# Denopia/canonical-k-mer-hash-table

Measured on AMD Instinct MI355X. Metric: k-mers/s inserted (canonical) + achieved HBM GB/s, 1/2/4/8 MI355X, higher is better.
Workload: dtype u64; 1 GPU; C2: synthetic 10000000 x 150 bp reads/GPU, k=31, -m 2 -s 200000000; reads_per_gpu=10000000, read_len=150, k=31, genome=50000000, table=-m 2 -s 200000000, parallelism=single

## Files before the change

canonical-k-mer-hash-table_amd/csrc/kc_count_impl.h:

```cpp
#pragma once
#include <algorithm>
#include <cstdlib>
#include <cstring>

#include "kc_common.h"

namespace kc {

static __constant__ uint64_t c_bf_seeds[MAX_NH] = {2411, 3253, 1061, 1129, 2269, 7309, 3491, 8237, 6359, 8779};

template <int W>
DEV bool table_insert(const TableView& tv, const uint64_t (&tk)[W], uint64_t add = 1) {
    constexpr int S = BUCKET_WORDS / (W + 1);
    const uint64_t region = region_of(tk[0], tv.R);
    uint32_t b = bucket_in_region(tk[0], tv.R);
    for (int probe = 0; probe < BPR; probe++) {
        uint64_t* bk = tv.buckets + (region * BPR + b) * BUCKET_WORDS;
        uint64_t w0[S];
        if constexpr (W == 1) {
            const uint4* b4 = reinterpret_cast<const uint4*>(bk);
#pragma unroll
            for (int q = 0; q < S / 2; q++) {
                uint4 v = b4[q];
                w0[2 * q] = ((uint64_t)v.y << 32) | v.x;
// ... 208 lines not shown
    return all;
}

DEV void block_add4(unsigned long long v0, unsigned long long v1, unsigned long long v2, unsigned long long v3,
                    unsigned long long* d0, unsigned long long* d1, unsigned long long* d2,
                    unsigned long long* d3) {
    __shared__ unsigned long long s_red[4][16];
    unsigned long long v[4] = {v0, v1, v2, v3};
    const int lane = threadIdx.x & 63, wid = threadIdx.x >> 6;
#pragma unroll
    for (int q = 0; q < 4; q++) {
        unsigned long long x = v[q];
        for (int d = 32; d >= 1; d >>= 1) x += __shfl_xor(x, d, 64);
        if (lane == 0) s_red[q][wid] = x;
    }
    __syncthreads();
    if (threadIdx.x < 4) {
        unsigned long long x = 0;
        for (int w = 0; w < (int)(blockDim.x / 64); w++) x += s_red[threadIdx.x][w];
        unsigned long long* dst = threadIdx.x == 0 ? d0 : threadIdx.x == 1 ? d1 : threadIdx.x == 2 ? d2 : d3;
        if (x && dst) atomicAdd(dst, x);
    }
}

template <int W>
constexpr int run_w() { return run_width(W); }
template <int W>
constexpr int tile_win() { return COUNT_THREADS * run_w<W>(); }
template <int W>
constexpr int scatter_threads() { return scatter_threads_w(W); }
template <int W, int NT>
constexpr int k1_runw() { return NT == scatter_threads_w(W) ? p1_runw(W) : run_w<W>(); }
template <int W, int OW, int NT>
constexpr size_t p1_smem(uint32_t F) { return bin_lds_bytes(F) + (size_t)NT * k1_runw<W, NT>() * 8 * OW; }
template <int W, int NT>
constexpr int k1_stage_words() { return NT * k1_runw<W, NT>() / 32 + W + 3; }
template <int W, int NT>
constexpr size_t p1_stage_smem() { return (size_t)k1_stage_words<W, NT>() * 24; }
template <int W>
constexpr int p2f_threads() { return p2f_threads_w(W); }

template <int W>
DEV bool window_tkey(const PackedView& sv, uint64_t p, const RollConst& rk, uint64_t (&tk)[W]) {
    uint64_t fwd[W], rc[W], key[W];
    if (!extract_window<W>(sv, p, rk, fwd)) return false;
    revcomp<W>(fwd, rk, rc);
    canonical<W>(fwd, rc, key);
    to_tkey<W>(key, tk);
    return true;
}

template <int W, int RUNW = run_w<W>(), class F>
DEV void tile_rolled(const PackedView& sv, uint64_t t0, uint64_t t1, const RollConst& rk, F&& f) {
    const uint64_t r0 = t0 + (uint64_t)threadIdx.x * RUNW, r1 = min(r0 + RUNW, t1);
    if (r0 < r1) {
        const uint64_t ps = r0 >= (uint64_t)(rk.k - 1) ? r0 - (rk.k - 1) : 0;
        roll_run<W, true>(sv, ps, r0, r1, rk, f);
    }
}

template <int W, int MODE>
__global__ __launch_bounds__(COUNT_THREADS) void k_count(PackedView sv, int k, TableView tv, BloomView bf,
                                                         DevCounters* __restrict__ ctr, uint64_t pow5_k,
                                                         uint64_t pow5_km1) {
    constexpr int TW = tile_win<W>();
    const uint64_t M = ctr->stream_len;
    const uint64_t t0 = (uint64_t)blockIdx.x * TW;
// ... 198 lines not shown
            const uint64_t pos = s_spbase + l.sp[b] + (i - lim);
            if (pos < o.spill_cap) {
                uint64_t* r = o.spill + pos * (W + o.rec);
#pragma unroll
                for (int w = 0; w < W; w++) r[w] = key[w];
                if (o.rec) r[W] = 1;
            } else {
                atomicOr(o.overflow, 1ULL);
            }
        }
    }
    __syncthreads();
    for (uint32_t b = tid; b < F; b += NT) {
        l.gbase[b] += l.lim[b];
        l.hist[b] = 0;
    }
    __syncthreads();
    return false;
}

DEV void scatter_seg_init(const PartLds& l, uint32_t b, uint64_t first) {
    l.hist[b] = 0;
    l.lim[b] = 0;
    l.gbase[b] = first;
}
DEV uint64_t scatter_seg_next(const PartLds& l, uint32_t b) { return l.gbase[b] + l.lim[b]; }

struct StoreWords {
    template <int W>
    DEV void operator()(uint64_t* __restrict__ out, uint64_t dst, const uint64_t (&key)[W], uint32_t) const {
#pragma unroll
        for (int w = 0; w < W; w++) ks_store(out + dst * W + w, key[w]);
    }
};
DEV uint64_t region_xlo(uint64_t r, uint64_t R) { return ((r << 32) + R - 1) / R; }
struct StoreRec6 {
    const uint32_t* xlo;
    DEV void operator()(uint64_t* __restrict__ out, uint64_t dst, const uint64_t (&key)[1], uint32_t b) const {
        uint32_t* q = reinterpret_cast<uint32_t*>(out) + (dst >> 1) * 3;
        q[dst & 1] = (uint32_t)key[0];
        reinterpret_cast<uint16_t*>(q + 2)[dst & 1] = (uint16_t)((uint32_t)(key[0] >> 32) - xlo[b]);
    }
};
struct Rec12 {
    int hb, xb;
    DEV uint3 enc(uint64_t t0, uint64_t t1) const {
        const uint32_t x = (uint32_t)(t0 >> 32), d = x & ((1u << xb) - 1);
        const uint32_t hi = ((uint32_t)(t1 >> 32) & ((1u << hb) - 1)) | (uint32_t)((t1 >> 62) & 1) << hb;
        return make_uint3((uint32_t)t0, (uint32_t)t1, hi | d << (hb + 1));
    }
    DEV void dec(uint3 r, uint32_t x0, uint64_t& t0, uint64_t& t1) const {
        const uint32_t x = x0 + (((r.z >> (hb + 1)) - x0) & ((1u << xb) - 1));
        t0 = ((uint64_t)x << 32) | r.x;
        t1 = ((uint64_t)(r.z & ((1u << hb) - 1)) << 32) | r.y | ((uint64_t)((r.z >> hb) & 1) << 62);
    }
};
struct StoreW2 {
    bool rec12;
    Rec12 rc;
    DEV void operator()(uint64_t* __restrict__ out, uint64_t dst, const uint64_t (&key)[2], uint32_t) const {
        if (rec12) {
            reinterpret_cast<uint3*>(out)[dst] = rc.enc(key[0], key[1]);
        } else {
            ks_store(out + dst * 2, key[0]);
            ks_store(out + dst * 2 + 1, key[1]);
        }
    }
};

template <int W, int RUNW, class Bin, class Out, int NT, class Mid = NoMid, class St = StoreWords, class Pre = NoMid>
DEV void scatter_seg(const PartLds& l, uint32_t F, const Bin& bin, const Out& o, uint64_t (&tk)[RUNW][W],
                     bool (&ok)[RUNW], uint64_t* __restrict__ out, Mid&& mid = Mid(),
                     const St& store = St(), Pre&& pre = Pre()) {
    static_assert(NT * RUNW <= 65536, "ranks ride in 16 bits");
    __shared__ unsigned long long s_spbase;
    __shared__ uint32_t s_spills, s_n;
    const int tid = threadIdx.x, lane = tid & 63;
    uint32_t pk[RUNW];
#pragma unroll
    for (int j = 0; j < RUNW; j++) {
        const uint32_t b = bin(tk[j][0]);
        if constexpr (W >= 2) {
            const uint32_t rk = atomicAdd(&l.hist[b], ok[j] ? 1u : 0u);
            pk[j] = ok[j] ? (b << 16) | rk : ~0u;
        } else {
            pk[j] = ok[j] ? (b << 16) | atomicAdd(&l.hist[b], 1u) : ~0u;
        }
    }
    pre();
    __syncthreads();
    if (tid < 64) {
        if (F % 4 == 0) {
            const uint32_t per = (F / 4 + 63) / 64, lo = min(F / 4, lane * per), hi = min(F / 4, lo + per);
            const uint4* h4 = reinterpret_cast<const uint4*>(l.hist);
            uint4* s4 = reinterpret_cast<uint4*>(l.start);
            uint32_t sum = 0;
#pragma unroll 1
            for (uint32_t i = lo; i < hi; i++) {
                const uint4 v = h4[i];
                sum += v.x + v.y + v.z + v.w;
            }
            const uint32_t incl = wave_incl_sum(sum);
            uint32_t run = incl - sum;
#pragma unroll 1
            for (uint32_t i = lo; i < hi; i++) {
                const uint4 v = h4[i];
                s4[i] = make_uint4(run, run + v.x, run + v.x + v.y, run + v.x + v.y + v.z);
                run += v.x + v.y + v.z + v.w;
            }
            if (lane == 63) s_n = incl;
        } else {
            const uint32_t per = (F + 63) / 64, lo = min(F, lane * per), hi = min(F, lo + per);
            uint32_t sum = 0;
#pragma unroll 1
            for (uint32_t i = lo; i < hi; i++) sum += l.hist[i];
            const uint32_t incl = wave_incl_sum(sum);
            uint32_t run = incl - sum;
#pragma unroll 1
            for (uint32_t i = lo; i < hi; i++) {
                l.start[i] = run;
                run += l.hist[i];
            }
            if (lane == 63) s_n = incl;
        }
        if (Out::kSeg && lane == 0) s_spills = 0;
    }
    __syncthreads();
#pragma unroll
    for (int j = 0; j < RUNW; j++)
        if (pk[j] != ~0u) {
            const uint32_t slot = l.start[pk[j] >> 16] + (pk[j] & 0xFFFFu);
#pragma unroll
            for (int w = 0; w < W; w++) l.keys[slot * W + w] = tk[j][w];
        }
    bool spills = false;
#pragma unroll 1
    for (uint32_t b = tid; b < F; b += NT) {
        const uint32_t st = l.start[b], h = l.hist[b];
        const uint64_t g = l.gbase[b] + l.lim[b];
        const uint32_t fit = (uint32_t)min((uint64_t)h, o.room(b, g));
        l.gbase[b] = g - st;
        l.lim[b] = st + fit;
        l.sp[b] = h - fit;
        l.hist[b] = 0;
        spills |= fit < h;
    }
    if (Out::kSeg && spills) s_spills = 1;
    mid();
    __syncthreads();
    if constexpr (Out::kSeg) {
        if (s_spills) {
            const uint32_t last = l.sp[F - 1];
            block_excl_scan_lds<NT>(l.sp, l.sp, F);
            if (tid == 0) s_spbase = atomicAdd(o.spill_n, (unsigned long long)(l.sp[F - 1] + last));
            __syncthreads();
        }
    }
    const uint32_t n = s_n;
    auto emit = [&](uint32_t i, const uint64_t (&key)[W], uint32_t b, uint32_t lim, uint64_t g) {
        if (i < lim) {
            store(out, g + i, key, b);
        } else if constexpr (Out::kSeg) {
            const uint64_t pos = s_spbase + l.sp[b] + (i - lim);
            if (pos < o.spill_cap) {
                uint64_t* r = o.spill + pos * (W + o.rec);
#pragma unroll
                for (int w = 0; w < W; w++) r[w] = key[w];
                if (o.rec) r[W] = 1;
            } else {
                atomicOr(o.overflow, 1ULL);
            }
        }
    };
#pragma unroll 1
    for (uint32_t i0 = tid; i0 < n; i0 += 2 * NT) {
        const uint32_t i1 = i0 + NT;
        const bool has1 = i1 < n;
        uint64_t k0[W], k1[W];
#pragma unroll
        for (int w = 0; w < W; w++) {
            k0[w] = l.keys[i0 * W + w];
            k1[w] = l.keys[(has1 ? i1 : i0) * W + w];
        }
        const uint32_t b0 = bin(k0[0]), b1 = bin(k1[0]);
        const uint32_t lim0 = l.lim[b0], lim1 = l.lim[b1];
        const uint64_t g0 = l.gbase[b0], g1 = l.gbase[b1];
        emit(i0, k0, b0, lim0, g0);
        if (has1) emit(i1, k1, b1, lim1, g1);
    }
}

constexpr bool bloom_mode(int MODE) { return MODE == 3 || MODE == 5; }

constexpr int HT = 64;
template <int OW>
constexpr size_t heavy_smem() { return (size_t)HT * (OW + 1) * 8; }
struct HeavyTab {
    uint64_t* keys;
    uint64_t* cnt;
};
template <int OW>
DEV HeavyTab heavy_tab(uint8_t* p) {
    HeavyTab h;
    h.keys = reinterpret_cast<uint64_t*>(p);
    h.cnt = h.keys + HT * OW;
    return h;
// ... 117 lines not shown
        const uint64_t c = h.cnt[e] & CNT_MASK;
        const bool has = key[0] != EMPTY;
        skew_append<OW, MODE>(pb, ctr, has, key, c);
        const uint64_t nrec = __ballot(has);
        if (threadIdx.x == 0 && nrec) atomicAdd(&ctr->heavy_n, (unsigned long long)__popcll(nrec));
    }
}

DEV bool gated_off(const unsigned long long* gate) { return gate && *gate == 0; }

constexpr int p1_out_words(int W, int MODE) { return MODE == 3 ? 1 : W; }
constexpr int scatter_waves(int NT, int RUNW, int OW, int cap) {
    const int wg = (int)(LDS_BYTES / ((size_t)NT * RUNW * 8 * OW));
    const int w = (wg < 1 ? 1 : wg) * NT / 256;
    return w < 1 ? 1 : w > cap ? cap : w;
}


template <int W, int MODE, bool SCATTER, class Bin, class Out, int NT = COUNT_THREADS>
__global__ __launch_bounds__(NT, scatter_waves(NT, k1_runw<W, NT>(), p1_out_words(W, MODE), 4)) void k_p1(PackedView sv, int k, BloomView bf,
                                                      DevCounters* __restrict__ ctr, PartBufs pb, uint32_t F, Bin bin_arg,
                                                      uint64_t* __restrict__ out, uint64_t pow5_k, uint64_t pow5_km1,
                                                      Out o, const unsigned long long* gate, int count) {
    extern __shared__ __attribute__((aligned(16))) uint8_t smem[];
    const Bin bin = level1_bins(bin_arg);
    constexpr int RUNW = k1_runw<W, NT>(), TW = NT * RUNW;
    constexpr bool COUNTS = !SCATTER || Out::kSeg;
    constexpr bool ROLLED = MODE == 2;
    constexpr int OW = p1_out_words(W, MODE);
    if (gated_off(gate)) return;
    if (gate && !SCATTER && blockIdx.x == 0 && threadIdx.x == 0) atomicAdd(&ctr->part_fallbacks, 1ULL);
    const PartLds l = part_lds(smem, F);
    constexpr bool HEAVY = Out::kSeg && !Bin::kOwner && !ROLLED;
    const HeavyTab ht = heavy_tab<OW>(smem + p1_smem<W, OW, NT>(F));
    if constexpr (HEAVY) {
        heavy_clear(ht, OW);
        for (int i = threadIdx.x; i < HT; i += NT) ht.cnt[i] = 0;
    }
    const int tid = threadIdx.x;
    const uint64_t M = ctr->stream_len;
    const uint64_t per = ((M + pb.nblk1 - 1) / pb.nblk1 + TW - 1) / TW * TW;
    const uint64_t lo = min(M, (uint64_t)blockIdx.x * per), hi = min(M, lo + per);
    constexpr bool STAGE = Out::kSeg && !ROLLED;
    constexpr int SW = k1_stage_words<W, NT>();
    static_assert(!STAGE || SW <= NT, "one stage word per thread");
    uint64_t* st_pk = reinterpret_cast<uint64_t*>(smem + p1_smem<W, OW, NT>(F) + heavy_smem<OW>());
    uint32_t* st_bk = reinterpret_cast<uint32_t*>(st_pk + 2 * SW);
    const uint64_t wlim = M ? ((M - 1) >> 5) + 1 : 0;
    auto stage_word = [&](uint64_t ts, int i, uint64_t& pw, uint32_t& bw) {
        const int64_t w = (int64_t)(ts >> 5) - (W + 1) + i;
        const bool in = w >= 0 && (uint64_t)w <= wlim;
        pw = in ? sv.pk[w] : 0;
        bw = in ? sv.bk[w] : 0;
    };
    if constexpr (STAGE)
        if (lo < hi && tid < SW) stage_word(lo, tid, st_pk[tid], st_bk[tid]);
    int par = 0;
    Out ob = o;
    if constexpr (Out::kSeg) ob.base = (uint64_t)blockIdx.x * o.cap;
    for (uint32_t b = tid; b < F; b += NT) {
        if constexpr (Out::kSeg) {
            scatter_seg_init(l, b, ob.start(b));
        } else {
            l.hist[b] = 0;
            if constexpr (SCATTER) l.gbase[b] = pb.off1[(uint64_t)b * pb.nblk1 + blockIdx.x];
        }
    }
    __syncthreads();
    const RollConst rk = make_roll<W>(k, pow5_k, pow5_km1);
    uint32_t n_win = 0, n_ins = 0;
    for (uint64_t t0 = lo; t0 < hi; t0 += TW) {
        const uint64_t t1 = min(t0 + TW, hi);
        uint64_t tk[RUNW][OW];
        bool ok[RUNW];
        if constexpr (!ROLLED) {
            const uint64_t r0 = t0 + (uint64_t)tid * RUNW;
#pragma unroll
            for (int j = 0; j < RUNW; j++) ok[j] = false;
            auto emit = [&](int j, bool valid, const uint64_t (&fwd)[W], const uint64_t (&rc)[W]) {
// ... 28 lines not shown
                canonical<W>(fwd, rc, key);
                to_tkey<W>(key, t);
                if (!bloom_gate(bf, root, t[0])) return;
                if constexpr (COUNTS) n_ins++;
#pragma unroll
                for (int j = 0; j < RUNW; j++)
                    if (!ok[j]) {
                        ok[j] = true;
#pragma unroll
                        for (int w = 0; w < W; w++) tk[j][w] = t[w];
                        break;
                    }
            });
        }
        if constexpr (SCATTER) {
            if constexpr (Out::kSeg) {
                const bool nxt = STAGE && t0 + TW < hi && tid < SW;
                uint64_t npk = 0;
                uint32_t nbk = 0;
                auto mid = [&]() {
                    if (nxt) {
                        st_pk[(par ^ 1) * SW + tid] = npk;
                        st_bk[(par ^ 1) * SW + tid] = nbk;
                    }
                };
                auto pre = [&]() {
                    if (nxt) stage_word(t0 + TW, tid, npk, nbk);
                };
                if constexpr (OW == 2)
                    scatter_seg<OW, RUNW, Bin, Out, NT>(l, F, bin, ob, tk, ok, out, mid,
                                                        StoreW2{(pb.rec12 & R12_P1) != 0, Rec12{pb.r12_hb, pb.r12_xb1}},
                                                        pre);
                else
                    scatter_seg<OW, RUNW, Bin, Out, NT>(l, F, bin, ob, tk, ok, out, mid, StoreWords(), pre);
                par ^= 1;
            } else {
                scatter_tile<OW, RUNW, Bin, Out, NT>(l, F, bin, ob, tk, ok, out, NoMid());
            }
        } else {
#pragma unroll
            for (int j = 0; j < RUNW; j++)
                if (ok[j]) atomicAdd(&l.hist[bin(tk[j][0])], 1u);
        }
    }
    if constexpr (!SCATTER) {
        __syncthreads();
        for (uint32_t b = tid; b < F; b += NT) pb.hist1[(uint64_t)b * pb.nblk1 + blockIdx.x] = l.hist[b];
    }
    if constexpr (Out::kSeg) {
        __syncthreads();
        for (uint32_t b = tid; b < F; b += NT)
            pb.hist1[(uint64_t)b * pb.nblk1 + blockIdx.x] = (uint32_t)(scatter_seg_next(l, b) - ob.start(b));
    }
    if constexpr (HEAVY) heavy_flush<OW, MODE>(ht, pb, ctr);
    if constexpr (COUNTS)
        if (count) {
            if constexpr (bloom_mode(MODE))
                block_add4(n_win, 0, 0, 0, &ctr->bf_windows, nullptr, nullptr, nullptr);
            else
                block_add4(n_win, Bin::kOwner ? 0 : n_ins, 0, 0, &ctr->windows, &ctr->inserted, nullptr, nullptr);
        }
}

struct DevN {
    const unsigned long long* dn;
    uint64_t cap;
    const unsigned long long* ovf;
// ... 170 lines not shown
            const uint64_t i = t0 + tid + (uint64_t)q * COUNT_THREADS;
            ok[q] = i < hi;
            const uint64_t ii = ok[q] ? i : lo;
#pragma unroll
            for (int w = 0; w < W; w++) tk[q][w] = pb.keys1[ii * W + w];
        }
        if constexpr (SCATTER) {
            scatter_tile<W, RUNW>(l, F, bin, OutExact{}, tk, ok, pb.keys2);
        } else {
#pragma unroll
            for (int q = 0; q < RUNW; q++)
                if (ok[q]) atomicAdd(&l.hist[bin(tk[q][0])], 1u);
        }
    }
    if constexpr (!SCATTER) {
        __syncthreads();
        for (uint32_t b = tid; b < F; b += COUNT_THREADS) pb.hist2[(rbase + b) * pb.B2 + j] = l.hist[b];
    }
}

template <int W, int NT>
constexpr size_t p2f_smem(uint32_t F, uint32_t nseg_max) { return part_smem<W, NT>(F) + (size_t)(nseg_max + 1) * 4; }

template <int W, int NT, int IS = W, bool REC6 = false>
__global__ __launch_bounds__(NT, scatter_waves(NT, run_w<W>(), W, 2048 / NT > 8 ? 8 : 2048 / NT)) void k_p2f(TableView tv, PartBufs pb, DevCounters* __restrict__ ctr,
                                                          int REC) {
    static_assert(!REC6 || W == 1, "6-byte records hold one-word keys");
    extern __shared__ __attribute__((aligned(16))) uint8_t smem[];
    constexpr int RUNW = run_w<W>(), TW = NT * RUNW;
    if (ctr->part_overflow) return;
    const uint32_t F = tv.F2;
    const BinRegion bin{tv.R, tv.f2bits, F - 1, 0};
    const PartLds l = part_lds(smem, F);
    uint32_t* pre = reinterpret_cast<uint32_t*>(smem + part_smem<W, NT>(F));
    const int tid = threadIdx.x;
    const uint32_t c = blockIdx.x / pb.B2, j = blockIdx.x % pb.B2;
    const uint32_t s_lo = (uint32_t)((uint64_t)j * pb.nblk1 / pb.B2);
    const uint32_t nseg = (uint32_t)((uint64_t)(j + 1) * pb.nblk1 / pb.B2) - s_lo;
    const uint64_t seg0 = (uint64_t)c * pb.nblk1 + s_lo;
    const uint32_t B2T = pb.b2t ? pb.b2t : pb.B2, jo = pb.b2off + j;
    const OutSeg o{(uint64_t)B2T * pb.cap2, ((uint64_t)c * F * B2T + jo) * pb.cap2, pb.cap2,
                   pb.spill, pb.spill_cap, &ctr->spill_n, &ctr->part_overflow, REC};
    for (uint32_t i = tid; i <= nseg; i += NT) pre[i] = i < nseg ? pb.hist1[seg0 + i] : 0;
    uint32_t* xlo = pre + nseg + 1;
    if constexpr (REC6)
        for (uint32_t b = tid; b < F; b += NT) xlo[b] = (uint32_t)region_xlo((uint64_t)c * F + b, tv.R);
    for (uint32_t b = tid; b < F; b += NT) scatter_seg_init(l, b, o.start(b));
    __syncthreads();
    block_excl_scan_lds<NT>(pre, pre, nseg + 1);
    const uint32_t total = pre[nseg];
    uint32_t cs = 0, cb = 0, nb = nseg ? pre[1] : 0;
    const bool rin = W == 2 && (pb.rec12 & R12_IN), rout = W == 2 && (pb.rec12 & R12_OUT);
    const uint32_t x0c = rin ? (uint32_t)region_xlo((uint64_t)c * F, tv.R) : 0;
    const uint64_t* sp = pb.keys1 + seg0 * pb.cap1 * IS;
    const uint32_t wpos = (uint32_t)(tid >> 6) * (64 * RUNW) + (tid & 63);
    auto load_tile = [&](uint32_t t0, uint64_t (&tk)[RUNW][W], bool (&ok)[RUNW]) {
#pragma unroll
        for (int q = 0; q < RUNW; q++) {
            const uint32_t i = t0 + wpos + q * 64;
            ok[q] = i < total;
            const uint64_t* src = sp;
            uint64_t item = (seg0 + cs) * pb.cap1;
            if (ok[q]) {
                if (nb <= i) {
                    do {
                        cs++;
                        cb = nb;
// ... 6 lines not shown
            }
            if constexpr (W == 2) {
                const uint64_t off = rin ? item * 12 : item * (8 * IS);
                uint32_t v[4];
                __builtin_memcpy(v, reinterpret_cast<const uint8_t*>(pb.keys1) + off, 16);
                tk[q][0] = v[0] | (uint64_t)v[1] << 32;
                tk[q][1] = v[2] | (uint64_t)v[3] << 32;
                (void)src;
                continue;
            }
#pragma unroll
            for (int w = 0; w < W; w++) tk[q][w] = ks_load(src + w);
        }
    };
    uint64_t tk[RUNW][W];
    bool ok[RUNW];
    if (total) load_tile(0, tk, ok);
    for (uint32_t t0 = 0; t0 < total; t0 += TW) {
        const bool more = t0 + TW < total;
        auto mid = [&]() {
            if (more) load_tile(t0 + TW, tk, ok);
        };
        if constexpr (W == 2) {
            if (rin) {
                const Rec12 r1{pb.r12_hb, pb.r12_xb1};
#pragma unroll
                for (int q = 0; q < RUNW; q++) {
                    const uint3 v = make_uint3((uint32_t)tk[q][0], (uint32_t)(tk[q][0] >> 32), (uint32_t)tk[q][1]);
                    r1.dec(v, x0c, tk[q][0], tk[q][1]);
                }
            }
        }
        if constexpr (REC6) {
            scatter_seg<W, RUNW, BinRegion, OutSeg, NT>(l, F, bin, o, tk, ok, pb.keys2, mid,
                                                        StoreRec6{xlo});
        } else if constexpr (W == 2) {
            scatter_seg<W, RUNW, BinRegion, OutSeg, NT>(l, F, bin, o, tk, ok, pb.keys2, mid,
                                                        StoreW2{rout, Rec12{pb.r12_hb, pb.r12_xb2}});
        } else {
            scatter_seg<W, RUNW, BinRegion, OutSeg, NT>(l, F, bin, o, tk, ok, pb.keys2, mid);
        }
    }
    __syncthreads();
    for (uint32_t b = tid; b < F; b += NT)
        pb.hist2[((uint64_t)c * F + b) * B2T + jo] = (uint32_t)(scatter_seg_next(l, b) - o.start(b));
}

DEV uint32_t lds_chunk(uint32_t b, uint32_t q) { return b * 8 + (q ^ ((b >> 1) & 7)); }
DEV uint64_t* lds_word(uint64_t* lt, uint32_t b, uint32_t word) {
    return lt + lds_chunk(b, word >> 1) * 2 + (word & 1);
}

DEV uint32_t slot_tag(uint64_t t0) { return 1u + (((uint32_t)t0 & 0xFFu) * 255u >> 8); }
DEV uint32_t zero_byte_mask4(uint32_t x) {
    const uint32_t z = ~(((x & 0x7F7F7F7Fu) + 0x7F7F7F7Fu) | x | 0x7F7F7F7Fu);
    return ((z >> 7) * 0x01020408u) >> 24;
}
DEV uint32_t zero_byte_mask8(uint64_t x) {
    return zero_byte_mask4((uint32_t)x) | zero_byte_mask4((uint32_t)(x >> 32)) << 4;
}

DEV void seg_prefix(uint32_t* s_pre, const uint32_t* __restrict__ fill, uint32_t n, uint32_t* s_pp = nullptr) {
    if (threadIdx.x < 64) {
        const uint32_t j = 2 * threadIdx.x;
        const uint32_t a = j < n ? fill[j] : 0, b = j + 1 < n ? fill[j + 1] : 0;
        const uint32_t inc = wave_incl_sum(a + b);
        const uint32_t ex = inc - (a + b);
        if (j < n) s_pre[j] = ex;
// ... 921 lines not shown
    hipLaunchKernelGGL(kh, dim3(pb.nblk1), dim3(COUNT_THREADS), sm1h, s, sym, k, bf, ctr, pb, F, bin, out, pk, pkm1,
                       OutExact{}, gate, count);
    launch_scan(pb.hist1, (uint64_t)F * pb.nblk1, pb.off1, pb.bsum, s, gate);
    hipLaunchKernelGGL(ks, dim3(pb.nblk1), dim3(COUNT_THREADS), sm1, s, sym, k, bf, ctr, pb, F, bin, out, pk, pkm1,
                       OutExact{}, gate, 0);
    return hipGetLastError();
}

template <int W, bool GATE>
static hipError_t insert_spill(TableView t, BloomView bf, DevCounters* ctr, PartBufs pb, hipStream_t s) {
    constexpr int IW = W + 1;
    const BinRegion bin = coarse_bins(t);
    const size_t sm1 = part_smem<IW>(t.F1), sm1h = hist_smem(t.F1);
    hipError_t e;
    if ((e = set_smem(k_p1k<IW, false>, sm1h)) != hipSuccess) return e;
    if ((e = set_smem(k_p1k<IW, true>, sm1)) != hipSuccess) return e;
    const DevN dn{&ctr->spill_n, pb.spill_cap, &ctr->part_overflow};
    hipLaunchKernelGGL((k_p1k<IW, false>), dim3(pb.nblk1), dim3(COUNT_THREADS), sm1h, s, pb.spill, (uint64_t)0, pb,
                       t.F1, bin, ctr, W, dn, IW);
    launch_scan(pb.hist1, (uint64_t)t.F1 * pb.nblk1, pb.off1, pb.bsum, s);
    hipLaunchKernelGGL((k_p1k<IW, true>), dim3(pb.nblk1), dim3(COUNT_THREADS), sm1, s, pb.spill, (uint64_t)0, pb,
                       t.F1, bin, ctr, W, dn, IW);
    return part_levels23<W, true, GATE>(t, ctr, pb, s, nullptr, 0, bf);
}

template <int W>
static hipError_t launch_p2f(TableView t, PartBufs pb, DevCounters* ctr, int rec, hipStream_t s, uint32_t pad = 0) {
    constexpr int NT = p2f_threads<W>(), NH = NT / 2;
    const uint32_t nseg = std::max<uint32_t>(pad, (pb.nblk1 + pb.B2 - 1) / pb.B2);
    hipError_t e;
    const size_t sm = p2f_smem<W, NT>(t.F2, nseg);
    if constexpr (W == 1) {
        if (pb.rec6) {
            if ((e = set_smem(k_p2f<1, NT, 1, true>, sm + (size_t)t.F2 * 4)) != hipSuccess) return e;
            hipLaunchKernelGGL((k_p2f<1, NT, 1, true>), dim3(t.F1 * pb.B2), dim3(NT), sm + (size_t)t.F2 * 4, s, t, pb,
                               ctr, rec);
            return hipGetLastError();
        }
    }
    if (sm <= LDS_BYTES || W <= 2) {
        if ((e = set_smem(k_p2f<W, NT>, sm)) != hipSuccess) return e;
        hipLaunchKernelGGL((k_p2f<W, NT>), dim3(t.F1 * pb.B2), dim3(NT), sm, s, t, pb, ctr, rec);
    } else {
        const size_t smh = p2f_smem<W, NH>(t.F2, nseg);
        if ((e = set_smem(k_p2f<W, NH>, smh)) != hipSuccess) return e;
        hipLaunchKernelGGL((k_p2f<W, NH>), dim3(t.F1 * pb.B2), dim3(NH), smh, s, t, pb, ctr, rec);
    }
    return hipGetLastError();
}

static __global__ void k_batch_begin(DevCounters* ctr) {
    ctr->part_overflow = 0;
    ctr->spill_n = 0;
    ctr->heavy_n = 0;
}
static __global__ void k_batch_end(DevCounters* ctr) {
    if (ctr->part_overflow) return;
    ctr->spilled += ctr->spill_n - ctr->heavy_n;
    ctr->heavy += ctr->heavy_n;
}

static inline void set_rec12_table(PartBufs& pb, const TableView& t, int k) {
    pb.rec12 = 0;
    if (t.R == 0) return;
    const int hb = std::max(0, 2 * k - 96);
    const uint64_t f2 = 1ULL << t.f2bits;
    const int xb1 = span_bits32(((f2 << 32) + t.R - 1) / t.R), xb2 = span_bits32(((1ULL << 32) + t.R - 1) / t.R);
    if (hb + 1 + xb1 <= 32) {
        pb.rec12 |= R12_P1 | R12_IN;
// ... 3 lines not shown
        pb.rec12 |= R12_OUT | R12_L2;
        pb.r12_xb2 = xb2;
    }
    if (pb.rec12) pb.rec12 |= R12_REG;
    pb.r12_hb = hb;
    pb.r12_b2s = 0;
}

template <int W, int MODE>
static hipError_t launch_part_w(PackedView sym, int k, TableView t, BloomView bf, DevCounters* ctr, PartBufs pb,
                                int fresh, hipStream_t s, int phase) {
    constexpr bool GATE3 = MODE == 4;
    if (pb.cap1 == 0) {
        if (!(phase & PH_MAIN)) return hipSuccess;
        hipError_t e = part_level1<W, MODE>(sym, k, bf, ctr, pb, t.F1, coarse_bins(t), pb.keys1, s);
        if (e != hipSuccess) return e;
        return part_levels23<W, false, GATE3>(t, ctr, pb, s, nullptr, fresh, bf);
    }
    hipError_t e;
    const unsigned long long* gate = &ctr->part_overflow;
    pb.rec6 = W == 1 && t.R >= (1ULL << 16);
    if constexpr (W == 2) set_rec12_table(pb, t, k);
    if (phase & PH_L3) {
        PartBufs p3 = pb;
        p3.B2 = pb.b2t;
        p3.b2t = p3.b2off = 0;
        if ((e = launch_p3<W, true, false, GATE3>(t, ctr, p3, nullptr, fresh, s, bf)) != hipSuccess) return e;
    }
    if (phase & (PH_MAIN | PH_L12)) {
    if (!pb.keep_skew) hipLaunchKernelGGL(k_batch_begin, dim3(1), dim3(1), 0, s, ctr);
    const uint64_t pk = pow5_mod54(k), pkm1 = pow5_mod54(k - 1);
    auto k1 = k_p1<W, MODE, true, BinRegion, OutSeg, scatter_threads<W>()>;
    const size_t p1_lds_min = (size_t)p1_tile(W) < 8 * (size_t)t.F1 ? LDS_BYTES / 2 + 16 : 0;
    const size_t sm1 = std::max(p1_lds_min, p1_smem<W, W, scatter_threads<W>()>(t.F1) + heavy_smem<W>() +
                                                p1_stage_smem<W, scatter_threads<W>()>());
    const OutSeg o1{(uint64_t)pb.nblk1 * pb.cap1, 0, pb.cap1, pb.spill, pb.spill_cap, &ctr->spill_n,
                    &ctr->part_overflow, 1};
    bool wide = false;
    if constexpr (W == 2) {
        if (p1_wide(W, t.F1)) {
            wide = true;
            auto kw = k_p1<W, MODE, true, BinRegion, OutSeg, P1_WIDE_THREADS>;
            const size_t smw = p1_smem<W, W, P1_WIDE_THREADS>(t.F1) + heavy_smem<W>() + p1_stage_smem<W, P1_WIDE_THREADS>();
            if ((e = set_smem(kw, smw)) != hipSuccess) return e;
            hipLaunchKernelGGL(kw, dim3(pb.nblk1), dim3(P1_WIDE_THREADS), smw, s, sym, k, bf, ctr, pb, t.F1,
                               coarse_bins(t), pb.keys1, pk, pkm1, o1, (const unsigned long long*)nullptr, 1);
        }
    }
    if (!wide) {
        if ((e = set_smem(k1, sm1)) != hipSuccess) return e;
        hipLaunchKernelGGL(k1, dim3(pb.nblk1), dim3(scatter_threads<W>()), sm1, s, sym, k, bf, ctr, pb, t.F1,
                           coarse_bins(t), pb.keys1, pk, pkm1, o1, (const unsigned long long*)nullptr, 1);
    }
    if ((e = launch_p2f<W>(t, pb, ctr, 1, s)) != hipSuccess) return e;
    if (phase & PH_MAIN)
        if ((e = launch_p3<W, true, false, GATE3>(t, ctr, pb, nullptr, fresh, s, bf)) != hipSuccess) return e;
    }
    if (!(phase & PH_TAIL)) return hipGetLastError();
    if ((e = insert_spill<W, GATE3>(t, bf, ctr, pb, s)) != hipSuccess) return e;
    hipLaunchKernelGGL(k_batch_end, dim3(1), dim3(1), 0, s, ctr);
    if ((e = part_level1<W, MODE>(sym, k, bf, ctr, pb, t.F1, coarse_bins(t), pb.keys1, s, gate)) != hipSuccess)
        return e;
    return part_levels23<W, false, GATE3>(t, ctr, pb, s, gate, fresh, bf);
}

template <int W>
static hipError_t count_part_w(PackedView sym, int k, int mode, TableView t, BloomView bf, DevCounters* ctr,
                               PartBufs pb, int fresh, hipStream_t s, int phase) {
// ... 493 lines not shown
```

canonical-k-mer-hash-table_amd/csrc/kc_internal.h:

```cpp
#pragma once
#include <hip/hip_runtime.h>
#include <stdint.h>

#include "../../include/kc_api.h"

namespace kc {

constexpr int TILE = 4096;
constexpr int TILE_THREADS = 256;
constexpr int COUNT_THREADS = 256;
constexpr int RUN = 32;
constexpr int BUCKET_WORDS = 16;
constexpr int BPR = 512;
constexpr uint64_t EMPTY = 0;
constexpr int BPR_BITS = 9;
constexpr uint64_t READY = 1ULL << 62;
constexpr uint64_t CNT_MASK = READY - 1;
constexpr int TEXT_T = 256;
constexpr int MAX_NH = 10;
constexpr uint8_t SYM_BREAK = 4;
constexpr int BF_BLOCKS_PER_REGION = 1024;
constexpr uint32_t RT_MAX_PARTS = 64;
constexpr uint32_t MAX_SEG_GROUP = 128;

// ... 96 lines not shown
    while (b < 32 && (1ULL << b) < span) b++;
    return b;
}
inline uint64_t level2_record_bytes(int W, int k, uint64_t R) {
    if (W == 1) return R >= (1ULL << 16) ? 6 : 8;
    if (W == 2 && R) {
        const int hb = 2 * k - 96 > 0 ? 2 * k - 96 : 0;
        if (hb + 1 + span_bits32(((1ULL << 32) + R - 1) / R) <= 32) return 12;
    }
    return 8ull * (uint64_t)W;
}

struct BloomView {
    uint32_t* bits;
    uint64_t mask;
    int nh;
    int nh_gate;
    int blocked;
    uint64_t nblocks;
    uint32_t slice_blocks;
};

constexpr int MAX_K = 479;
constexpr int MAX_W = 15;
inline int words_for_k(int k) { return k / 32 + 1; }
inline int slots_per_bucket(int W) { return BUCKET_WORDS / (W + 1); }

constexpr int run_width(int W) { return W == 1 ? 16 : W == 2 ? 8 : W <= 4 ? 8 : 4; }
constexpr int scatter_threads_w(int W) { return W <= 4 ? 512 : 256; }
constexpr int p1_runw(int W) { return run_width(W); }
constexpr int p1_tile(int W) { return scatter_threads_w(W) * p1_runw(W); }
constexpr size_t bin_lds_bytes(uint32_t F) { return ((size_t)F * 24 + 15) / 16 * 16 + 16; }
constexpr int p2f_threads_w(int W) { return W <= 2 ? 1024 : W <= 4 ? 512 : 256; }
constexpr size_t p1_stage_bytes(int W) { return (size_t)(p1_tile(W) / 32 + W + 3) * 24; }
constexpr size_t p1_lds_bytes(int W, uint32_t F1) {
    return bin_lds_bytes(F1) + (size_t)p1_tile(W) * 8 * W + (size_t)64 * (W + 1) * 8 + p1_stage_bytes(W);
}
constexpr size_t p2f_lds_bytes(int W, uint32_t F2, uint32_t nseg, int nt = 0) {
    return bin_lds_bytes(F2) + (size_t)(nt ? nt : p2f_threads_w(W)) * run_width(W) * 8 * W + ((size_t)nseg + 1) * 4;
}
constexpr size_t LDS_BYTES = 160 * 1024;
constexpr int P1_WIDE_THREADS = 1024;
constexpr size_t p1_lds_bytes_nt(int W, uint32_t F1, int nt) {
    return bin_lds_bytes(F1) + (size_t)nt * p1_runw(W) * 8 * W + (size_t)64 * (W + 1) * 8 +
           (size_t)(nt * p1_runw(W) / 32 + W + 3) * 24;
}
constexpr bool p1_wide(int W, uint32_t F1) {
    return W == 2 && (uint64_t)p1_tile(W) < 8ULL * F1 && p1_lds_bytes_nt(W, F1, P1_WIDE_THREADS) <= LDS_BYTES;
}
constexpr int p1_tile_max(int W) { return W == 2 ? P1_WIDE_THREADS * p1_runw(W) : p1_tile(W); }

hipError_t launch_tokenize(const uint8_t* src, uint64_t ntiles, const ChunkDesc* d_chunks, int n_chunks,
                           int fmt, TileInfo* tiles, TileOut* touts, TileOut* tblk, PackedView sv,
                           uint64_t sym_bound, DevCounters* ctr, hipStream_t s);
hipError_t launch_count(PackedView sv, uint64_t sym_bound, int k, int mode, TableView t, BloomView bf,
                        DevCounters* ctr, hipStream_t s);
constexpr int PH_MAIN = 1, PH_TAIL = 2, PH_ALL = 3;
constexpr int PH_L12 = 16, PH_L3 = 32;
hipError_t launch_count_partitioned(PackedView sv, uint64_t sym_bound, int k, int mode, TableView t,
                                    BloomView bf, DevCounters* ctr, PartBufs pb, int fresh, hipStream_t s,
                                    int phase = PH_ALL);
hipError_t launch_bloom_partitioned(PackedView sv, int k, int W, BloomView bf, TableView ft, TableView fg,
                                    DevCounters* ctr, PartBufs pb, int fresh, int keep, hipStream_t s,
                                    int phase = PH_ALL);
hipError_t launch_count_reuse(int W, TableView t, BloomView bf, DevCounters* ctr, PartBufs pb, int fresh, int level,
                              int gate, uint64_t windows, hipStream_t s);
hipError_t launch_bloom_records(int W, const uint64_t* rec, uint64_t n, BloomView bf, TableView ft, DevCounters* ctr,
                                PartBufs pb, int fresh, hipStream_t s);
hipError_t launch_count_records(int W, const uint64_t* rec, uint64_t n, TableView t, BloomView bf, DevCounters* ctr,
                                PartBufs pb, int fresh, int gate, hipStream_t s);
hipError_t launch_hold_overflow(DevCounters* ctr, int restore, hipStream_t s);
constexpr int CHECKSUM_SLOTS = 64;
// ... 141 lines not shown
```

Baseline: 87.76 billion k-mers/s.

## Align scattered one-word keys to global parity and store them as 16-byte pairs

For one-word keys in the pass-1 and pass-2 partition scatter, the per-bin LDS start offsets are now chosen with a parity-aware prefix scan (DPP-based) so each bin's staged keys match the parity of their global destination. Pairs of adjacent keys can then be written with a single 16-byte or 12-byte record store instead of two 8-byte stores. Leftover odd head and tail elements are handled separately, and zero-filled pad slots mark gaps. This adds LDS padding per bin, a more complex scan, and extra boundary handling, which may lower occupancy.

```diff
diff --git a/canonical-k-mer-hash-table_amd/csrc/kc_count_impl.h b/canonical-k-mer-hash-table_amd/csrc/kc_count_impl.h
--- a/canonical-k-mer-hash-table_amd/csrc/kc_count_impl.h
+++ b/canonical-k-mer-hash-table_amd/csrc/kc_count_impl.h
@@ -264,7 +264,11 @@
 template <int W, int NT>
 constexpr int k1_runw() { return NT == scatter_threads_w(W) ? p1_runw(W) : run_w<W>(); }
 template <int W, int OW, int NT>
-constexpr size_t p1_smem(uint32_t F) { return bin_lds_bytes(F) + (size_t)NT * k1_runw<W, NT>() * 8 * OW; }
+constexpr size_t p1_smem(uint32_t F, bool pair = false) {
+    return bin_lds_bytes(F) + (size_t)NT * k1_runw<W, NT>() * 8 * OW + (pair ? pair_pad_bytes(F) : 0);
+}
+template <int W, int MODE, int NT>
+constexpr bool p1_pair() { return KC_PAIR_L1 && W == 1 && MODE == 0 && NT == scatter_threads_w(W); }
 template <int W, int NT>
 constexpr int k1_stage_words() { return NT * k1_runw<W, NT>() / 32 + W + 3; }
 template <int W, int NT>
@@ -529,6 +533,9 @@
 #pragma unroll
         for (int w = 0; w < W; w++) ks_store(out + dst * W + w, key[w]);
     }
+    DEV void pair(uint64_t* __restrict__ out, uint64_t dst, uint64_t ka, uint64_t kb, uint32_t) const {
+        *reinterpret_cast<ulonglong2*>(out + dst) = make_ulonglong2(ka, kb);
+    }
 };
 DEV uint64_t region_xlo(uint64_t r, uint64_t R) { return ((r << 32) + R - 1) / R; }
 struct StoreRec6 {
@@ -537,6 +544,12 @@
         uint32_t* q = reinterpret_cast<uint32_t*>(out) + (dst >> 1) * 3;
         q[dst & 1] = (uint32_t)key[0];
         reinterpret_cast<uint16_t*>(q + 2)[dst & 1] = (uint16_t)((uint32_t)(key[0] >> 32) - xlo[b]);
+    }
+    DEV void pair(uint64_t* __restrict__ out, uint64_t dst, uint64_t ka, uint64_t kb, uint32_t b) const {
+        const uint32_t x = xlo[b];
+        const uint32_t da = ((uint32_t)(ka >> 32) - x) & 0xFFFFu, db = (uint32_t)(kb >> 32) - x;
+        *reinterpret_cast<uint3*>(reinterpret_cast<uint32_t*>(out) + (dst >> 1) * 3) =
+            make_uint3((uint32_t)ka, (uint32_t)kb, da | db << 16);
     }
 };
 struct Rec12 {
@@ -565,7 +578,17 @@
     }
 };
 
-template <int W, int RUNW, class Bin, class Out, int NT, class Mid = NoMid, class St = StoreWords, class Pre = NoMid>
+DEV uint32_t run_step(uint32_t f, uint32_t h, uint32_t g) {
+    if (!h) return f;
+    const uint32_t a0 = f & 0xFFFFu, a1 = f >> 16;
+    return (a0 + ((a0 ^ g) & 1) + h) | (a1 + ((a1 ^ g ^ 1) & 1) + h) << 16;
+}
+DEV uint32_t run_then(uint32_t f, uint32_t s) {
+    const uint32_t a0 = f & 0xFFFFu, a1 = f >> 16;
+    return (a0 + ((a0 & 1) ? s >> 16 : s & 0xFFFFu)) | (a1 + ((a1 & 1) ? s & 0xFFFFu : s >> 16)) << 16;
+}
+template <int W, int RUNW, class Bin, class Out, int NT, bool PAIR = false, class Mid = NoMid, class St = StoreWords,
+          class Pre = NoMid>
 DEV void scatter_seg(const PartLds& l, uint32_t F, const Bin& bin, const Out& o, uint64_t (&tk)[RUNW][W],
                      bool (&ok)[RUNW], uint64_t* __restrict__ out, Mid&& mid = Mid(),
                      const St& store = St(), Pre&& pre = Pre()) {
@@ -587,7 +610,63 @@
     pre();
     __syncthreads();
     if (tid < 64) {
-        if (F % 4 == 0) {
+        if constexpr (PAIR) {
+            static_assert(W == 1 && NT * RUNW <= 32768, "pairs of one-word keys; padded tile slots ride in 16 bits");
+            const bool quads = F % 4 == 0;
+            uint32_t ln = lane;
+            asm volatile("" : "+v"(ln));
+            const uint32_t nu = quads ? F / 4 : F, per = (nu + 63) / 64, lo = min(nu, ln * per), hi = min(nu, lo + per);
+            const uint4* h4 = reinterpret_cast<const uint4*>(l.hist);
+            auto par = [&](uint32_t b) { return ((uint32_t)l.gbase[b] + l.lim[b]) & 1u; };
+            auto par4 = [&](uint32_t i) {
+                const uint4 lm = reinterpret_cast<const uint4*>(l.lim)[i];
+                const uint4 ga = reinterpret_cast<const uint4*>(l.gbase)[2 * i];
+                const uint4 gb = reinterpret_cast<const uint4*>(l.gbase)[2 * i + 1];
+                return make_uint4((ga.x + lm.x) & 1u, (ga.z + lm.y) & 1u, (gb.x + lm.z) & 1u, (gb.z + lm.w) & 1u);
+            };
+            uint32_t f = 0;
+#pragma unroll 1
+            for (uint32_t i = lo; i < hi; i++) {
+                if (quads) {
+                    const uint4 v = h4[i], p = par4(i);
+                    f = run_step(run_step(run_step(run_step(f, v.x, p.x), v.y, p.y), v.z, p.z), v.w, p.w);
+                } else {
+                    f = run_step(f, l.hist[i], par(i));
+                }
+            }
+            f = run_then((uint32_t)__builtin_amdgcn_update_dpp(0, (int)f, 0x111, 0xF, 0xF, false), f);
+            f = run_then((uint32_t)__builtin_amdgcn_update_dpp(0, (int)f, 0x112, 0xF, 0xF, false), f);
+            f = run_then((uint32_t)__builtin_amdgcn_update_dpp(0, (int)f, 0x114, 0xF, 0xF, false), f);
+            f = run_then((uint32_t)__builtin_amdgcn_update_dpp(0, (int)f, 0x118, 0xF, 0xF, false), f);
+            f = run_then((uint32_t)__builtin_amdgcn_update_dpp(0, (int)f, 0x142, 0xA, 0xF, false), f);
+            f = run_then((uint32_t)__builtin_amdgcn_update_dpp(0, (int)f, 0x143, 0xC, 0xF, false), f);
+            const uint32_t ex = __shfl_up(f, 1, 64);
+            uint32_t run = lane ? ex & 0xFFFFu : 0;
+            auto place = [&](uint32_t h, uint32_t p) {
+                if (h) run += (run ^ p) & 1;
+                const uint32_t st = run;
+                run += h;
+                return st;
+            };
+#pragma unroll 1
+            for (uint32_t i = lo; i < hi; i++) {
+                if (quads) {
+                    const uint4 v = h4[i], p = par4(i);
+                    uint4 s;
+                    s.x = place(v.x, p.x);
+                    s.y = place(v.y, p.y);
+                    s.z = place(v.z, p.z);
+                    s.w = place(v.w, p.w);
+                    reinterpret_cast<uint4*>(l.start)[i] = s;
+                } else {
+                    l.start[i] = place(l.hist[i], par(i));
+                }
+            }
+            if (lane == 63) {
+                s_n = f & 0xFFFFu;
+                l.keys[f & 0xFFFFu] = 0;
+            }
+        } else if (F % 4 == 0) {
             const uint32_t per = (F / 4 + 63) / 64, lo = min(F / 4, lane * per), hi = min(F / 4, lo + per);
             const uint4* h4 = reinterpret_cast<const uint4*>(l.hist);
             uint4* s4 = reinterpret_cast<uint4*>(l.start);
@@ -641,6 +720,10 @@
         l.sp[b] = h - fit;
         l.hist[b] = 0;
         spills |= fit < h;
+        if constexpr (PAIR) {
+            if ((b + 1 < F ? l.start[b + 1] : s_n) != st + h) l.keys[st + h] = 0;
+            if (b == 0 && st) l.keys[0] = 0;
+        }
     }
     if (Out::kSeg && spills) s_spills = 1;
     mid();
@@ -669,6 +752,48 @@
             }
         }
     };
+    if constexpr (PAIR) {
+        const uint4* k4 = reinterpret_cast<const uint4*>(l.keys);
+        uint32_t t = tid;
+        asm volatile("" : "+v"(t));
+#pragma unroll 1
+        for (uint32_t i0 = 2 * t; i0 < n; i0 += 4 * NT) {
+            const uint32_t i1 = i0 + 2 * NT;
+            const bool has1 = i1 < n;
+            const uint4 q0 = k4[i0 >> 1], q1 = k4[(has1 ? i1 : i0) >> 1];
+            const uint64_t a0 = q0.x | (uint64_t)q0.y << 32, c0 = q0.z | (uint64_t)q0.w << 32;
+            const uint64_t a1 = q1.x | (uint64_t)q1.y << 32, c1 = q1.z | (uint64_t)q1.w << 32;
+            const uint32_t b0 = bin(a0), b1 = bin(a1);
+            const uint32_t lim0 = l.lim[b0], lim1 = l.lim[b1];
+            const uint64_t g0 = l.gbase[b0], g1 = l.gbase[b1];
+            if (a0 && i0 + 1 < lim0) store.pair(out, g0 + i0, a0, c0, b0);
+            if (has1 && a1 && i1 + 1 < lim1) store.pair(out, g1 + i1, a1, c1, b1);
+        }
+#pragma unroll 1
+        for (uint32_t b = t; b < F; b += NT) {
+            const uint32_t st = l.start[b], lim = l.lim[b];
+            const uint64_t g = l.gbase[b];
+            if (st < lim) {
+                if (st & 1) {
+                    const uint64_t key[1] = {l.keys[st]};
+                    store(out, g + st, key, b);
+                }
+                if (!(lim & 1)) continue;
+                const uint64_t key[1] = {l.keys[lim - 1]};
+                store(out, g + (lim - 1), key, b);
+            }
+        }
+        if (s_spills) {
+#pragma unroll 1
+            for (uint32_t i = t; i < n; i += NT) {
+                const uint64_t key[1] = {l.keys[i]};
+                if (!key[0]) continue;
+                const uint32_t b = bin(key[0]), lim = l.lim[b];
+                if (i >= lim) emit(i, key, b, lim, 0);
+            }
+        }
+        return;
+    }
 #pragma unroll 1
     for (uint32_t i0 = tid; i0 < n; i0 += 2 * NT) {
         const uint32_t i1 = i0 + NT;
@@ -852,7 +977,8 @@
     if (gate && !SCATTER && blockIdx.x == 0 && threadIdx.x == 0) atomicAdd(&ctr->part_fallbacks, 1ULL);
     const PartLds l = part_lds(smem, F);
     constexpr bool HEAVY = Out::kSeg && !Bin::kOwner && !ROLLED;
-    const HeavyTab ht = heavy_tab<OW>(smem + p1_smem<W, OW, NT>(F));
+    constexpr bool PAIR = SCATTER && Out::kSeg && !Bin::kOwner && p1_pair<W, MODE, NT>();
+    const HeavyTab ht = heavy_tab<OW>(smem + p1_smem<W, OW, NT>(F, PAIR));
     if constexpr (HEAVY) {
         heavy_clear(ht, OW);
         for (int i = threadIdx.x; i < HT; i += NT) ht.cnt[i] = 0;
@@ -864,7 +990,7 @@
     constexpr bool STAGE = Out::kSeg && !ROLLED;
     constexpr int SW = k1_stage_words<W, NT>();
     static_assert(!STAGE || SW <= NT, "one stage word per thread");
-    uint64_t* st_pk = reinterpret_cast<uint64_t*>(smem + p1_smem<W, OW, NT>(F) + heavy_smem<OW>());
+    uint64_t* st_pk = reinterpret_cast<uint64_t*>(smem + p1_smem<W, OW, NT>(F, PAIR) + heavy_smem<OW>());
     uint32_t* st_bk = reinterpret_cast<uint32_t*>(st_pk + 2 * SW);
     const uint64_t wlim = M ? ((M - 1) >> 5) + 1 : 0;
     auto stage_word = [&](uint64_t ts, int i, uint64_t& pw, uint32_t& bw) {
@@ -959,7 +1085,7 @@
                                                         StoreW2{(pb.rec12 & R12_P1) != 0, Rec12{pb.r12_hb, pb.r12_xb1}},
                                                         pre);
                 else
-                    scatter_seg<OW, RUNW, Bin, Out, NT>(l, F, bin, ob, tk, ok, out, mid, StoreWords(), pre);
+                    scatter_seg<OW, RUNW, Bin, Out, NT, PAIR>(l, F, bin, ob, tk, ok, out, mid, StoreWords(), pre);
                 par ^= 1;
             } else {
                 scatter_tile<OW, RUNW, Bin, Out, NT>(l, F, bin, ob, tk, ok, out, NoMid());
@@ -1196,7 +1322,8 @@
     const uint32_t F = tv.F2;
     const BinRegion bin{tv.R, tv.f2bits, F - 1, 0};
     const PartLds l = part_lds(smem, F);
-    uint32_t* pre = reinterpret_cast<uint32_t*>(smem + part_smem<W, NT>(F));
+    constexpr bool PAIR = REC6 && KC_PAIR_L2;
+    uint32_t* pre = reinterpret_cast<uint32_t*>(smem + part_smem<W, NT>(F) + (PAIR ? pair_pad_bytes(F) : 0));
     const int tid = threadIdx.x;
     const uint32_t c = blockIdx.x / pb.B2, j = blockIdx.x % pb.B2;
     const uint32_t s_lo = (uint32_t)((uint64_t)j * pb.nblk1 / pb.B2);
@@ -1269,8 +1396,8 @@
             }
         }
         if constexpr (REC6) {
-            scatter_seg<W, RUNW, BinRegion, OutSeg, NT>(l, F, bin, o, tk, ok, pb.keys2, mid,
-                                                        StoreRec6{xlo});
+            scatter_seg<W, RUNW, BinRegion, OutSeg, NT, PAIR>(l, F, bin, o, tk, ok, pb.keys2, mid,
+                                                              StoreRec6{xlo});
         } else if constexpr (W == 2) {
             scatter_seg<W, RUNW, BinRegion, OutSeg, NT>(l, F, bin, o, tk, ok, pb.keys2, mid,
                                                         StoreW2{rout, Rec12{pb.r12_hb, pb.r12_xb2}});
@@ -2258,9 +2385,9 @@
     const size_t sm = p2f_smem<W, NT>(t.F2, nseg);
     if constexpr (W == 1) {
         if (pb.rec6) {
-            if ((e = set_smem(k_p2f<1, NT, 1, true>, sm + (size_t)t.F2 * 4)) != hipSuccess) return e;
-            hipLaunchKernelGGL((k_p2f<1, NT, 1, true>), dim3(t.F1 * pb.B2), dim3(NT), sm + (size_t)t.F2 * 4, s, t, pb,
-                               ctr, rec);
+            const size_t sm6 = sm + (size_t)t.F2 * 4 + (KC_PAIR_L2 ? pair_pad_bytes(t.F2) : 0);
+            if ((e = set_smem(k_p2f<1, NT, 1, true>, sm6)) != hipSuccess) return e;
+            hipLaunchKernelGGL((k_p2f<1, NT, 1, true>), dim3(t.F1 * pb.B2), dim3(NT), sm6, s, t, pb, ctr, rec);
             return hipGetLastError();
         }
     }
@@ -2330,8 +2457,8 @@
     const uint64_t pk = pow5_mod54(k), pkm1 = pow5_mod54(k - 1);
     auto k1 = k_p1<W, MODE, true, BinRegion, OutSeg, scatter_threads<W>()>;
     const size_t p1_lds_min = (size_t)p1_tile(W) < 8 * (size_t)t.F1 ? LDS_BYTES / 2 + 16 : 0;
-    const size_t sm1 = std::max(p1_lds_min, p1_smem<W, W, scatter_threads<W>()>(t.F1) + heavy_smem<W>() +
-                                                p1_stage_smem<W, scatter_threads<W>()>());
+    const size_t sm1 = std::max(p1_lds_min, p1_smem<W, W, scatter_threads<W>()>(t.F1, p1_pair<W, MODE, scatter_threads<W>()>()) +
+                                                heavy_smem<W>() + p1_stage_smem<W, scatter_threads<W>()>());
     const OutSeg o1{(uint64_t)pb.nblk1 * pb.cap1, 0, pb.cap1, pb.spill, pb.spill_cap, &ctr->spill_n,
                     &ctr->part_overflow, 1};
     bool wide = false;
diff --git a/canonical-k-mer-hash-table_amd/csrc/kc_internal.h b/canonical-k-mer-hash-table_amd/csrc/kc_internal.h
--- a/canonical-k-mer-hash-table_amd/csrc/kc_internal.h
+++ b/canonical-k-mer-hash-table_amd/csrc/kc_internal.h
@@ -152,12 +152,21 @@
 constexpr int p1_tile(int W) { return scatter_threads_w(W) * p1_runw(W); }
 constexpr size_t bin_lds_bytes(uint32_t F) { return ((size_t)F * 24 + 15) / 16 * 16 + 16; }
 constexpr int p2f_threads_w(int W) { return W <= 2 ? 1024 : W <= 4 ? 512 : 256; }
+#ifndef KC_PAIR_L1
+#define KC_PAIR_L1 1
+#endif
+#ifndef KC_PAIR_L2
+#define KC_PAIR_L2 1
+#endif
+constexpr size_t pair_pad_bytes(uint32_t F) { return ((size_t)F + 2 + (F & 1)) * 8; }
 constexpr size_t p1_stage_bytes(int W) { return (size_t)(p1_tile(W) / 32 + W + 3) * 24; }
 constexpr size_t p1_lds_bytes(int W, uint32_t F1) {
-    return bin_lds_bytes(F1) + (size_t)p1_tile(W) * 8 * W + (size_t)64 * (W + 1) * 8 + p1_stage_bytes(W);
+    return bin_lds_bytes(F1) + (size_t)p1_tile(W) * 8 * W + (size_t)64 * (W + 1) * 8 + p1_stage_bytes(W) +
+           (W == 1 && KC_PAIR_L1 ? pair_pad_bytes(F1) : 0);
 }
 constexpr size_t p2f_lds_bytes(int W, uint32_t F2, uint32_t nseg, int nt = 0) {
-    return bin_lds_bytes(F2) + (size_t)(nt ? nt : p2f_threads_w(W)) * run_width(W) * 8 * W + ((size_t)nseg + 1) * 4;
+    return bin_lds_bytes(F2) + (size_t)(nt ? nt : p2f_threads_w(W)) * run_width(W) * 8 * W + ((size_t)nseg + 1) * 4 +
+           (W == 1 && KC_PAIR_L2 ? pair_pad_bytes(F2) : 0);
 }
 constexpr size_t LDS_BYTES = 160 * 1024;
 constexpr int P1_WIDE_THREADS = 1024;
```

After: 87.72 billion k-mers/s. About the same (-0.0%).
